# moss-lab/ScanFold

Hardware: AMD Instinct MI355X
Metric: windows/sec (W=120, step=1, 100 shuffles) (higher is better)
Workload: dtype int32 (int16 LDS storage) energies; f64 partition function

## Files before the change

scanfold_amd/csrc/sf_mfe_fast.hip.h:

```cpp
#pragma once
#include <type_traits>
#include "sf_energy.h"
#include "sf_pk16.h"

#define SF_FAST_NR 34
#ifndef SF_FAST_TINY_D0
#define SF_FAST_TINY_D0 10
#endif
#define SF_FAST_CHUNK_D0 36
#ifndef SF_FAST_UNPACK
#define SF_FAST_UNPACK 1
#endif
#ifndef SF_UNP_PB
#define SF_UNP_PB 4
#endif
#define SF_HELP_MERGE_MAXW 118
#define SF_DML_HELPER_BIAS_256 26
#define SF_DML_HELPER_BIAS_W200 50
#define SF_DML_HELPER_BIAS(ng, wt) ((ng) == 256 ? ((wt) == 200 ? SF_DML_HELPER_BIAS_W200 : SF_DML_HELPER_BIAS_256) : 100000)
#define SF_HELP_NB_128 4
#define SF_HELP_NB_128G 8
#define SF_HELP_NB_256 6
#define SF_INF16 30000
#define SF_FAST_THRESH 10000
// ... 799 lines not shown
  const int type = X.tPair[S[i] * 8 + S[j]];
  int ext;
  if (i > 1 && j < W) ext = tExt[SF_TIDX(type, S[i - 1], S[j + 1])];
  else if (i > 1) ext = X.tD5[type * 5 + S[i - 1]];
  else if (j < W) ext = X.tD3[type * 5 + S[j + 1]];
  else ext = 0;
  return v - ext - (type > 2 ? X.TAU : 0);
}

__device__ inline int sf_fast_traceback(const SfFastCtx &X, const int32_t *f5s, const int16_t *tExt, const int lane,
                                        int16_t *stI, int16_t *stJ, int16_t *stM, char *dbL) {
  const int W = X.W;
  const bool FOLD = X.fold != 0;
  const uint8_t *S = X.S;
  const SfDevParams *D = X.D;
#define TC(i, j) sf_fast_c(X, tExt, (i), (j))
#define TF(i, j) (((j) - (i) < SFD_TURN + 1) ? SF_INF16 : (int)X.fML[FBASE((j) - (i)) + (i)-1])
#define TPAIR(i, j) (((j) - (i)) <= X.maxd ? (int)X.tPair[S[i] * 8 + S[j]] : 0)
  for (int x = lane; x < W; x += 64) dbL[x] = '.';
  int sp = 0, bad = 0;
  stI[0] = 1; stJ[0] = (int16_t)W; stM[0] = 0; sp = 1;
  while (sp > 0 && !bad) {
    --sp;
    int i = stI[sp], j = stJ[sp];
    const int ml = stM[sp];
    bool have_pair = false;
    if (ml == 0) {
      while (j > 0 && f5s[j] == f5s[j - 1]) j--;
      if (j < SFD_TURN + 2) continue;
      const int fij = f5s[j];
      int found = -1;
      for (int base = j - SFD_TURN - 1; base >= 1 && found < 0; base -= 64) {
        const int k = base - lane;
        bool ok = false;
        if (k >= 1) {
          const int type = TPAIR(k, j);
          if (type) {
            int ext;
            if (k > 1 && j < W) ext = tExt[SF_TIDX(type, S[k - 1], S[j + 1])];
            else if (k > 1) ext = X.tD5[type * 5 + S[k - 1]];
            else if (j < W) ext = X.tD3[type * 5 + S[j + 1]];
            else ext = 0;
            ok = (fij == f5s[k - 1] + TC(k, j) + ext + (type > 2 ? X.TAU : 0));
          }
        }
        const unsigned long long m = __ballot(ok);
        if (m) found = base - (__ffsll(m) - 1);
      }
      if (found < 0) { bad = 1; break; }
      stI[sp] = 1; stJ[sp] = (int16_t)(found - 1); stM[sp] = 0; sp++;
      i = found;
      have_pair = true;
    } else {
      if (j - i < SFD_TURN + 1) { bad = 1; break; }
      while (j - i > SFD_TURN + 1 && TF(i, j - 1) < SF_INF16 && TF(i, j) == TF(i, j - 1) + X.MLbase) j--;
      while (j - i > SFD_TURN + 1 && TF(i + 1, j) < SF_INF16 && TF(i, j) == TF(i + 1, j) + X.MLbase) i++;
      const int fij = TF(i, j);
      const int type = TPAIR(i, j);
      int stem = 0;
      if (type) {
        if (i > 1 && j < W) stem = X.tM[SF_TIDX(type, S[i - 1], S[j + 1])];
        else if (i > 1) stem = X.tD5[type * 5 + S[i - 1]];
        else if (j < W) stem = X.tD3[type * 5 + S[j + 1]];
        stem += (type > 2 ? X.TAU : 0) + X.MLintern;
      }
      if (type && fij == TC(i, j) + stem) {
        have_pair = true;
      } else {
        int found = -1;
        for (int base = i + SFD_TURN + 1; base <= j - SFD_TURN - 2 && found < 0; base += 64) {
          const int k = base + lane;
          bool ok = false;
          if (k <= j - SFD_TURN - 2) {
            const int a = TF(i, k), b = TF(k + 1, j);
            ok = a < SF_INF16 && b < SF_INF16 && fij == a + b;
          }
          const unsigned long long m = __ballot(ok);
          if (m) found = base + (__ffsll(m) - 1);
        }
        if (found < 0) { bad = 1; break; }
        stI[sp] = (int16_t)i; stJ[sp] = (int16_t)found; stM[sp] = 1; sp++;
        stI[sp] = (int16_t)(found + 1); stJ[sp] = (int16_t)j; stM[sp] = 1; sp++;
      }
    }
    while (have_pair) {
      dbL[i - 1] = '(';
      dbL[j - 1] = ')';
      const int type = TPAIR(i, j);
      const int cij = TC(i, j);
      if (cij == sfd_hairpin(D, S, i, j, type)) break;
      const int d = j - i;
      const int umax = sfd_min(SFD_MAXLOOP, d - 2 - (SFD_TURN + 1));
      int found = -1;
      if (umax >= 0) {
        const int tmax = umax * 31 + umax;
        for (int base = 0; base <= tmax && found < 0; base += 64) {
          const int t = base + lane;
          const int u1 = t / 31, u2 = t - u1 * 31;
          bool ok = false;
          if (u1 + u2 <= umax) {
            const int p = i + 1 + u1, q = j - 1 - u2;
            const int t2 = TPAIR(p, q);
            if (t2)
              ok = (cij == sfd_intloop(D, u1, u2, type, sfd_rtype(t2), S[i + 1], S[j - 1], S[p - 1], S[q + 1]) + TC(p, q) +
                           ((X.sc && (u1 | u2) == 0) ? X.sc[i] + X.sc[i + 1] + X.sc[j - 1] + X.sc[j] : 0));
          }
          const unsigned long long m = __ballot(ok);
          if (m) found = base + (__ffsll(m) - 1);
        }
      }
      if (found >= 0) {
        const int u1 = found / 31, u2 = found - u1 * 31;
        i = i + 1 + u1;
        j = j - 1 - u2;
        continue;
      }
      const int tr = sfd_rtype(type);
      const int mm = X.MLclosing + X.tM[SF_TIDX(tr, S[j - 1], S[i + 1])] + (tr > 2 ? X.TAU : 0) + X.MLintern;
      int fk = -1;
      for (int base = i + 1 + SFD_TURN + 1; base <= j - 1 - SFD_TURN - 2 && fk < 0; base += 64) {
        const int k = base + lane;
        bool ok = false;
        if (k <= j - 1 - SFD_TURN - 2) {
          const int a = TF(i + 1, k), b = TF(k + 1, j - 1);
          ok = a < SF_INF16 && b < SF_INF16 && cij == a + b + mm;
        }
        const unsigned long long m = __ballot(ok);
        if (m) fk = base + (__ffsll(m) - 1);
      }
      if (fk < 0) { bad = 1; break; }
      stI[sp] = (int16_t)(i + 1); stJ[sp] = (int16_t)fk; stM[sp] = 1; sp++;
      stI[sp] = (int16_t)(fk + 1); stJ[sp] = (int16_t)(j - 1); stM[sp] = 1; sp++;
      break;
    }
  }
#undef TC
#undef TF
#undef TPAIR
  return bad;
}


template <int NQ>
__device__ __forceinline__ void sf_fast_exterior(const SfFastCtx &X, const int W, const int lane, const int seq,
                                                 int32_t *f5s, const int16_t *tExt, const int16_t *etab,
                                                 const int32_t *flag,
                                                 int16_t *stack_area, char *dbL, int32_t *__restrict__ out,
                                                 int *__restrict__ ovf_cnt, int *__restrict__ ovf_list,
                                                 const int trace_stride, char *__restrict__ db_out,
                                                 int *__restrict__ status) {
  const uint8_t *S = X.S;
  const uint8_t *tPair = X.tPair;
  int P[NQ], sj[NQ], sj1[NQ];
#pragma unroll
  for (int q = 0; q < NQ; q++) {
    const int j = lane + 64 * q + 1;
    P[q] = SF_FAST_BIG * 2;
    sj[q] = j <= W ? S[j] : 0;
    sj1[q] = j <= W ? S[j + 1] : 0;
  }
  int f5prev = 0;
  const bool want_trace = db_out && (seq % trace_stride) == 0;
  if (lane == 0) f5s[0] = 0;
  auto column_min = [&](const int jf) -> int {
    const int l = (jf - 1) & 63, q = (jf - 1) >> 6;
    int v = SF_LANE_READ(P[0], l);
#pragma unroll
    for (int qq = 1; qq < NQ; qq++) {
      const int vq = SF_LANE_READ(P[qq], l);
      if (q == qq) v = vq;
    }
    return v;
  };
  constexpr int PF = 8;
  int cb[PF][NQ];
  auto load_row = [&](const int i, int(&dst)[NQ]) {
#pragma unroll
    for (int q = 0; q < NQ; q++) {
      const int j = lane + 64 * q + 1;
      dst[q] = (i <= W - SFD_TURN - 1 && j <= W && i + SFD_TURN + 1 <= j) ? (int)(etab ? etab : X.cg)[SF_CGIDX(i, j)] : SF_INF16;
    }
  };
#pragma unroll
  for (int k = 0; k < PF; k++) load_row(1 + k, cb[k]);
#pragma unroll 1
  for (int i0 = 1; i0 <= W - SFD_TURN - 1; i0 += PF) {
#pragma unroll
    for (int k = 0; k < PF; k++) {
      const int i = i0 + k;
      if (i <= W - SFD_TURN - 1) {
        if (i >= 2) {
          f5prev = sfd_min(f5prev, column_min(i - 1));
          if (want_trace && lane == 0) f5s[i - 1] = f5prev;
        }
        if (etab || X.cg_ext) {
#pragma unroll
          for (int q = 0; q < NQ; q++) P[q] = sfd_min(P[q], f5prev + cb[k][q]);
        } else {
        const int si = S[i], sim1 = S[i - 1];
#pragma unroll
        for (int q = 0; q < NQ; q++) {
          const int j = lane + 64 * q + 1;
          if (j <= W && i + SFD_TURN + 1 <= j) {
            const int type = j - i <= X.maxd ? tPair[si * 8 + sj[q]] : 0;
            if (type) {
              int ext;
              if (i > 1 && j < W) ext = tExt[SF_TIDX(type, sim1, sj1[q])];
              else if (i > 1) ext = X.tD5[type * 5 + sim1];
              else if (j < W) ext = X.tD3[type * 5 + sj1[q]];
              else ext = 0;
              P[q] = sfd_min(P[q], f5prev + cb[k][q] + ext + (type > 2 ? X.TAU : 0));
            }
          }
        }
        }
        load_row(i + PF, cb[k]);
      }
    }
  }
  for (int jf = sfd_max(W - SFD_TURN - 1, 1); jf <= W; jf++) {
    f5prev = sfd_min(f5prev, column_min(jf));
    if (want_trace && lane == 0) f5s[jf] = f5prev;
  }
  SF_WAVE_SYNC();
  const int over = flag[0] || f5prev < SF_FAST_OVF;
  if (lane == 0) {
    out[seq] = f5prev;
    if (over) {
      const int k = atomicAdd(ovf_cnt, 1);
      ovf_list[k] = seq;
    }
  }
  if (db_out && !over && (seq % trace_stride) == 0) {
    int16_t *stI = stack_area;
    int16_t *stJ = stI + W + 8;
    int16_t *stM = stJ + W + 8;
    const int bad = sf_fast_traceback(X, f5s, tExt, lane, stI, stJ, stM, dbL);
    char *dst = db_out + (size_t)(seq / trace_stride) * (W + 1);
    for (int x = lane; x <= W; x += 64) dst[x] = x < W ? dbL[x] : 0;
    if (bad && lane == 0) atomicOr(status, 1);
  }
}

#define SF_DEFER_ROWS_256 3
template <int NQ>
struct SfTrail {
  int F[NQ];
  int f3n;
  int row;
};
template <int NQ>
__device__ __forceinline__ void sf_trail_load(const int16_t *cgp, const int W, const int lane, const int i, int (&c)[NQ]) {
#pragma unroll
  for (int q = 0; q < NQ; q++) {
    const int j = lane + 1 + 64 * q;
    c[q] = (i >= 1 && j <= W && i + SFD_TURN + 1 <= j) ? (int)cgp[SF_CGIDX(i, j)] : SF_INF16;
  }
}
template <int NQ>
__device__ __forceinline__ void sf_trail_row(SfTrail<NQ> &T, const int lane, const int i, const int (&c)[NQ]) {
  if (i < 1) return;
  int m = c[0] + T.F[0];
#pragma unroll
  for (int q = 1; q < NQ; q++) m = sfd_min(m, c[q] + T.F[q]);
  T.f3n = sfd_min(T.f3n, sf_wave_min(m));
  if (i >= 2) {
    const int l = (i - 2) & 63, h = (i - 2) >> 6;
#pragma unroll
    for (int q = 0; q < NQ; q++) T.F[q] = (lane == l && h == q) ? T.f3n : T.F[q];
  }
}
template <int NQ, int NR>
__device__ __forceinline__ void sf_trail_rows(SfTrail<NQ> &T, const int lane, const int nrows, const int (&c)[NR][NQ]) {
#pragma unroll
  for (int k = 0; k < NR; k++)
    if (k < nrows) sf_trail_row<NQ>(T, lane, T.row - k, c[k]);
  T.row -= nrows;
}
template <int NQ>
__device__ __forceinline__ void sf_trail_result(const SfTrail<NQ> &T, const int lane, const int seq, const int over,
                                                int32_t *__restrict__ out, int *__restrict__ ovf_cnt,
                                                int *__restrict__ ovf_list) {
  if (lane == 0) {
    out[seq] = T.f3n;
    if (over || T.f3n < SF_FAST_OVF) {
      const int k = atomicAdd(ovf_cnt, 1);
      ovf_list[k] = seq;
    }
  }
}


enum SfStep {
  SF_STEP_SIZED,
  SF_STEP_GUARDED,
  SF_STEP_UNSPLIT,
  SF_STEP_SPLIT,
  SF_STEP_SPLIT16,
  SF_STEP_SPLIT8,
  SF_STEP_NARROW,
};
template <SfStep K>
using SfStepTag = std::integral_constant<SfStep, K>;

__device__ __forceinline__ int16_t sf_poison16(const int poison, const int x) {
  const int k = poison == 5 ? 1 + (int)(((uint32_t)x * 2654435761u) >> 30) : poison;
  return (int16_t)(k == 1 ? -32768 : (k == 2 ? -28000 : (k == 3 ? 0 : 32767)));
}

template <int NG, int WT, bool MG = false, bool HC = false, bool PZ = false>
__global__ __launch_bounds__(2 * NG, SF_FAST_WAVES_PER_SIMD) void sf_mfe_fast_kernel(const uint8_t *__restrict__ seqs, int n, int Wrt,
                                                             const SfDevParams *__restrict__ D,
                                                             const SfFastParams *__restrict__ F,
                                                             const SfFastRows *__restrict__ Rows,
                                                             int16_t *__restrict__ cg_all, int32_t *__restrict__ out,
                                                             int *__restrict__ ovf_cnt, int *__restrict__ ovf_list,
                                                             int trace_stride, char *__restrict__ db_out,
                                                             int *__restrict__ status, int *__restrict__ work_ctr,
                                                             const char *__restrict__ cons_rows,
                                                             const int32_t *__restrict__ sc_rows, int poison) {
  constexpr int NT = 2 * NG;
  constexpr bool FOLD = (NG == 256);
  const int W = WT ? WT : Wrt;
  SF_DYN_SMEM(smem);
  const SfFastLayout Lo = sf_fast_layout(W, HC);
  SfFastCtx X;
  char *const hcC = (char *)(smem + Lo.off_hc);
  uint8_t *const hcP = (uint8_t *)hcC + (W + 2), *const hcE = hcP + (W + 2);
  int16_t *const scS = (int16_t *)(smem + Lo.off_hc + (((3 * (W + 2)) + 1) & ~1));
  X.hc.c = (HC && cons_rows) ? hcC : nullptr; X.hc.partner = hcP; X.hc.encl = hcE;
  X.sc = (HC && sc_rows) ? scS : nullptr;
  X.fML = (int16_t *)smem;
  X.CI = (int16_t *)(smem + Lo.off_ci);
  X.C1N = nullptr; X.CB = nullptr;
  X.BN = (int16_t *)(smem + Lo.off_c1n);
#ifdef SF_EMUL
  sf_emul_bn_base = (const char *)X.BN; sf_emul_ci_base = (const char *)X.CI;
#endif
  X.DMLr = nullptr;
  int16_t *tab = (int16_t *)(smem + Lo.off_tab);
  X.t23 = tab; X.tI = tab + 175 - 25; X.t1n = tab + 325 - 25; X.tM = tab + 475 - 25; X.tH = tab + 625 - 25;
  X.tE = tab + 775 - 25; X.cg_ext = 1;
  X.tStack = tab + 925; X.tD5 = tab + 989; X.tD3 = tab + 1029;
  uint8_t *tPair = (uint8_t *)(tab + 1069);
  X.tPair = tPair;
  uint8_t *tRPair = (uint8_t *)(tab + SF_FAST_TAB_OLD);
  int16_t *t23in = tab + SF_FAST_TAB_OLD + 32;
  X.tRPair = tRPair; X.t23in = t23in;
  int32_t *flag = (int32_t *)(smem + Lo.off_flag);
  uint8_t *S = (uint8_t *)(smem + Lo.off_S);
  X.S = S;
  X.D = D; X.F = F; X.R = Rows; X.W = W; X.fold = FOLD; X.maxd = D->max_pair_dist;
  constexpr bool MERGE = MG && (NG == 128);
  constexpr bool UNPK = SF_FAST_UNPACK && (NG == 128);
  constexpr bool LGLOOPS = MG && (NG == 128);
  constexpr int TBLK = WT > 0 ? 1 : (NG == 128 ? (MG ? 2 : 1) : 0);
  X.bn_dup = (NG == 128);
  uint8_t *const cell_list = (MG && W >= SF_HELP_MERGE_MAXW) ? (uint8_t *)((int16_t *)(smem + Lo.off_tab) + 1069 + 32 + 1)
                                                            : (uint8_t *)(smem + Lo.off_list);
  X.TAU = D->P.TerminalAU; X.MLbase = D->P.MLbase; X.MLclosing = D->P.MLclosing; X.MLintern = D->P.MLintern[1];
  int32_t *f5s = (int32_t *)(smem + Lo.off_ci);
  int16_t *tExt = (int16_t *)(smem + Lo.off_ci + (((W + 1) * 4 + 3) & ~3));

  const int tid = threadIdx.x;
  X.cg = cg_all + (size_t)sf_fast_scratch_slot(blockIdx.x, gridDim.x) * SF_CG_ENTRIES(W);
  for (int x = tid; x < 175; x += NT) {
    tab[x] = F->mm23[x];
    if (x < 150) {
      tab[175 + x] = F->mmI[25 + x]; tab[325 + x] = F->mm1n[25 + x]; tab[475 + x] = F->mmM[25 + x];
      tab[625 + x] = F->mmH[25 + x]; tab[775 + x] = F->mmExt[25 + x];
    }
  }
  for (int x = tid; x < 175; x += NT) t23in[x] = F->mm23in[x];
  for (int x = tid; x < 64; x += NT) { tab[925 + x] = F->stackT[x]; tPair[x] = F->pair[x]; tRPair[x] = F->rpair[x]; }
  for (int x = tid; x < 40; x += NT) { tab[989 + x] = F->d5[x]; tab[1029 + x] = F->d3[x]; }

  {
    int16_t *uni = tab + 1069 + 32 + 1;
    X.uNIN = uni;
    for (int x = tid; x < 128; x += NT) uni[x] = F->uni[x];
  }
  const int grp = SF_WAVE_UNIFORM(tid / NG);
  const int tg = tid - grp * NG;
  constexpr int CENTRE = (NG == 256) ? 128 : 32;
  constexpr bool SHARE = SF_DML_HELPER_BIAS(NG, WT) < 10000;
  constexpr bool DML2 = (NG == 128);
  const int OFFs = ((W + 1) >> 1) - CENTRE;
  const int OFF = (NG > 64) ? (OFFs + NG) & (NG - 1) : 0;
  const int v = (tg + OFF) & (NG - 1);
  constexpr int MAIN_LO = (NG == 256) ? 64 : 0, MAIN_HI = (NG == 256) ? 191 : 63;
  const bool can_split = (NG == 128 && W >= 64) || NG == 256;
  const int split_d0 = can_split ? ((sfd_max(sfd_max(SFD_MAXLOOP + 6, 2 * (MAIN_LO - 1 + OFFs)), 2 * (W - OFFs - MAIN_HI)) + 1) & ~1) : 1 << 30;
  constexpr bool NARROW = (NG == 256);
  const int narrow_d0 = (NARROW && can_split && W >= 168)
                            ? sfd_max(split_d0, (sfd_max(2 * (96 - 1 + OFFs), 2 * (W - OFFs - 159)) + 1) & ~1) : 1 << 30;

  constexpr int NQ = NG / 64;
  const bool sweeper = SF_WAVE_UNIFORM(tid >> 6) == (NG == 128 ? 3 : 7);
  const int n_split_steps = split_d0 < W ? (W - split_d0 + 1) / 2 : 0;
  constexpr int DROWS = (NG == 128 || WT != 200) ? 4 : SF_DEFER_ROWS_256;
  const int defer_need = n_split_steps > 0 ? (W - SFD_TURN - 1 + n_split_steps - 1) / n_split_steps : 0;
  const int defer_rows = sfd_min(defer_need, DROWS);
  const bool defer_on = n_split_steps >= 8 && defer_need <= 4;
  SfTrail<NQ> T;
#pragma unroll
  for (int q = 0; q < NQ; q++) T.F[q] = 0;
  T.f3n = 0; T.row = 0;

  int *const next_slot = (int *)(smem + Lo.off_next);
  int seq = blockIdx.x;
  while (seq < n) {
    const uint8_t *src = seqs + (size_t)seq * W;
    constexpr bool PINF = true;
    int tidf = tid;
    if (PINF) SF_PIN(tidf);
    __syncthreads();
    if (PZ) {
      for (int x = tid; x < Lo.off_tab / 2; x += NT) ((int16_t *)smem)[x] = sf_poison16(poison, x);
      if (HC) for (int x = tid; x < (Lo.total - Lo.off_hc) / 2; x += NT) ((int16_t *)(smem + Lo.off_hc))[x] = sf_poison16(poison, x);
      __syncthreads();
    }
    for (int x = tidf; x < W; x += NT) S[x + 1] = sf_encode_nt(src[x]);
    if (MG && W >= SF_HELP_MERGE_MAXW) for (int x = tidf; x < 128; x += NT) ((int16_t *)(smem + Lo.off_tab) + 1069 + 32 + 1)[x] = F->uni[x];
    for (int x = tidf; x < (Lo.off_tab - Lo.off_ci) / 4; x += NT) ((uint32_t *)X.CI)[x] = sf_pk(SF_INF16, SF_INF16);
    int fetched = 0;
    if (tid == 0) {
      S[0] = 0; S[W + 1] = 0; flag[0] = 0;
      fetched = (int)gridDim.x + atomicAdd(work_ctr, 1);
    }
    __syncthreads();
    if (HC) {
      if (cons_rows)
        for (int x = tid; x < W; x += NT) hcC[x + 1] = cons_rows[(size_t)seq * W + x];
      if (sc_rows)
        for (int x = tid; x < W; x += NT) scS[x + 1] = (int16_t)sfd_max(sfd_min(sc_rows[(size_t)seq * W + x], 30000), -30000);
      __syncthreads();
      if (cons_rows && tid == 0) flag[0] = sf_hc_parse8(W, hcC, hcP, hcE) ? 2 : 0;
      __syncthreads();
      if (cons_rows && flag[0] == 2) {
        if (tid == 0) { atomicOr(status, 2); out[seq] = 0; *next_slot = fetched; }
        __syncthreads();
        seq = *next_slot;
        continue;
      }
    }
    int next_seq = n;
    const bool trail_this = defer_on && !(db_out && (seq % trace_stride) == 0);
    if (sweeper) {
#pragma unroll
      for (int q = 0; q < NQ; q++) T.F[q] = 0;
      T.f3n = 0; T.row = trail_this ? W - SFD_TURN - 1 : 0;
    }
    int ovf = 0;
    uint32_t H[14];
    int dprev = SF_INF16;
    int fnb = SF_FAST_BIG;
#pragma unroll
    for (int k = 0; k < 14; k++) H[k] = (uint32_t)SF_INF16 | ((uint32_t)SF_INF16 << 16);

    int slot2 = (SFD_TURN + 1 + grp - 2) % SF_FAST_NR, slotd = (SFD_TURN + 1 + grp) % SF_FAST_NR;
    auto build_list = [&](const int dd0) {
      const int lane = tid & 63;
      const int d1 = dd0 + 1;
      const int iH = ((v - 64) & (NG - 1)) - (dd0 >> 1);
      const bool vA = (dd0 < W) && (iH >= 1) && (iH + dd0 <= W), vB = (d1 < W) && (iH >= 1) && (iH + d1 <= W);
      const int tA = (vA && dd0 <= X.maxd) ? X.tPair[S[iH] * 8 + S[iH + dd0]] : 0;
      const int tB = (vB && d1 <= X.maxd) ? X.tPair[S[iH] * 8 + S[iH + d1]] : 0;
      const unsigned long long mA = __ballot(tA != 0), mB = __ballot(tB != 0);
      const int cA = __popcll(mA);
      uint8_t *list = cell_list + (((dd0 >> 1) & 1) << 7);
      const unsigned long long below = (1ull << lane) - 1ull;
      if (tA) list[__popcll(mA & below)] = (uint8_t)iH;
      if (tB) list[cA + __popcll(mB & below)] = (uint8_t)(iH | 128);
      if (lane == 0) list[127] = (uint8_t)(cA + __popcll(mB));
    };
    SfHU HU;
    auto step = [&](const int d0, auto kind_tag) {
      constexpr SfStep KIND = decltype(kind_tag)::value;
      constexpr int LGC = KIND == SF_STEP_SPLIT16 ? 4 : (KIND == SF_STEP_SPLIT8 ? 3 : (KIND == SF_STEP_SPLIT && LGLOOPS ? 5 : 0));
      constexpr bool DO_G = KIND == SF_STEP_SIZED, DO_CH = KIND == SF_STEP_GUARDED;
      const int d = d0 + grp;
      if (d0 == SFD_TURN + 1 + 2 && tid == 0) *next_slot = fetched;
      if (d0 == SFD_TURN + 1 + 4) next_seq = SF_WAVE_UNIFORM(*next_slot);
      constexpr bool split = KIND >= SF_STEP_SPLIT;
      constexpr bool narrow = KIND == SF_STEP_NARROW;
      if (NARROW && d0 == narrow_d0) {
        uint32_t *const xa = (uint32_t *)X.BN;
        const int RWc = W - 4;
        if (tg >= 96 && tg < 160) {
#pragma unroll
          for (int k = 0; k < 14; k++) xa[(grp * 16 + k) * RWc + 100 + (tg - 96)] = H[k];
          xa[(grp * 16 + 14) * RWc + 100 + (tg - 96)] = (uint32_t)dprev;
          xa[(grp * 16 + 15) * RWc + 100 + (tg - 96)] = (uint32_t)fnb;
        }
        __syncthreads();
        if (tg >= 64 && tg < 128) {
#pragma unroll
          for (int k = 0; k < 14; k++) H[k] = xa[(grp * 16 + k) * RWc + 100 + (tg - 64)];
          dprev = (int)xa[(grp * 16 + 14) * RWc + 100 + (tg - 64)];
          fnb = (int)xa[(grp * 16 + 15) * RWc + 100 + (tg - 64)];
        }
        __syncthreads();
      }
      const bool helper = split && (NG == 256 ? (narrow ? tg < 64 : (tg < 64 || tg >= 192)) : tg >= 64);
      const int vh = NG == 256 ? (narrow ? v + 96 : (tg < 64 ? v + 64 : v - 64)) : v - 64;
      const int vm = narrow ? ((v + 32) & (NG - 1)) : v;
      constexpr bool DML4 = NARROW && (WT == 200);
      const bool dmlw = DML4 && narrow && tg >= 128;
      const int vd = tg >= 192 ? v - 96 : v - 32;
      const int i = (NARROW && !DML4 && narrow && tg >= 128) ? -1
                    : ((dmlw ? (vd & (NG - 1)) : (helper ? (vh & (NG - 1)) : vm)) - (d >> 1));
      const int dml_terms = d - 2 * SFD_TURN - 2;
      const int dml_cut = d - SFD_TURN - 1 - sfd_max(sfd_min(dml_terms / 2 - SF_DML_HELPER_BIAS(NG, WT), dml_terms), 0);
      const bool valid = (d < W) && (i >= 1) && (i + d <= W);
      int fpart = SF_FAST_BIG;
      int dec = SF_FAST_BIG, eh = SF_FAST_BIG, e0 = SF_FAST_BIG;
      SfPub pub;
      pub.a = pub.b = 0; pub.tau = 0; pub.type = 0;
      int dc[DROWS][NQ];
      const bool sweep_now = defer_on && sweeper && split && T.row > 0;
      const int sweep_rows = sweep_now ? sfd_max(sfd_min(defer_rows, T.row - (W - d0)), 0) : 0;
      if (sweep_now) {
#pragma unroll
        for (int k = 0; k < DROWS; k++)
          if (k < sweep_rows) sf_trail_load<NQ>(X.cg, W, tid & 63, T.row - k, dc[k]);
      }
      if (__ballot(valid)) {
        if (DO_G && d0 < 8) sf_fast_cell<true, WT, SF_SEC_ALL, false, FOLD, 1>(X, d, i, valid, slot2, slotd, H, HU, ovf, grp == 0, fnb, fpart, dec, eh, e0, dprev, pub);
        else if (DO_G && d0 < SF_FAST_TINY_D0) sf_fast_cell<true, WT, SF_SEC_ALL, false, FOLD, 5>(X, d, i, valid, slot2, slotd, H, HU, ovf, grp == 0, fnb, fpart, dec, eh, e0, dprev, pub);
        else if (DO_CH && d0 < SF_FAST_CHUNK_D0) sf_fast_cell<false, WT, SF_SEC_ALL, true, FOLD, SFD_MAXLOOP, TBLK>(X, d, i, valid, slot2, slotd, H, HU, ovf, grp == 0, fnb, fpart, dec, eh, e0, dprev, pub);
        else if (!split) sf_fast_cell<false, WT, SF_SEC_ALL, false, FOLD, SFD_MAXLOOP, TBLK, false, UNPK && KIND == SF_STEP_UNSPLIT>(X, d, i, valid, slot2, slotd, H, HU, ovf, grp == 0, fnb, fpart, dec, eh, e0, dprev, pub);
        else if (DML4 && narrow) {
          const int nmain = dml_terms / 5, cA = SFD_TURN + 1 + nmain, cB = cA + (dml_terms - nmain + 1) / 2;
          uint32_t *const xa = (uint32_t *)X.BN;
          if (dmlw) {
            const bool wB = tg >= 192;
            sf_fast_cell<false, WT, SF_SEC_DML, false, FOLD, SFD_MAXLOOP, TBLK>(X, d, i, valid, slot2, slotd, H, HU, ovf, false, fnb, fpart, dec, eh, e0, dprev, pub, wB ? cB : cA, wB ? (1 << 20) : cB - 1);
            if (valid) xa[(grp * 16 + (wB ? 1 : 0)) * (W - 4) + 100 + (tg & 63)] = (uint32_t)sfd_min(dec, 32000);
          } else if (!helper) {
            sf_fast_cell<false, WT, SF_SEC_P1 | SF_SEC_C0 | SF_SEC_DML | SF_SEC_PRE, false, FOLD, SFD_MAXLOOP, TBLK>(X, d, i, valid, slot2, slotd, H, HU, ovf, grp == 0, fnb, fpart, dec, eh, e0, dprev, pub, SFD_TURN + 1, cA - 1);
          } else {
            sf_fast_cell<false, WT, SF_SEC_HELP, false, FOLD, SFD_MAXLOOP, TBLK>(X, d, i, valid, slot2, slotd, H, HU, ovf, grp == 0, fnb, fpart, dec, eh, e0, dprev, pub);
            if (valid) X.BN[2 * (slotd * (W - 4) + i - 1)] = (int16_t)sfd_min(eh, 32000);
          }
        }
        else if (!helper) {
          if (SHARE) sf_fast_cell<false, WT, SF_SEC_P1 | SF_SEC_C0 | SF_SEC_DML | SF_SEC_PRE, false, FOLD, SFD_MAXLOOP, TBLK>(X, d, i, valid, slot2, slotd, H, HU, ovf, grp == 0, fnb, fpart, dec, eh, e0, dprev, pub, SFD_TURN + 1, dml_cut - 1);
          else {
            static_assert(SHARE || DML2, "a main wave either shares the multiloop split with its helpers (NG = 256) or runs it two cells per lane (NG = 128)");
            dec = sf_fast_dml2<WT, LGC>(X, d, tid & 63, i, valid);
            sf_fast_cell<false, WT, SF_SEC_P1 | SF_SEC_C0 | SF_SEC_PRE, false, FOLD, SFD_MAXLOOP, TBLK, false, UNPK && split>(X, d, i, valid, slot2, slotd, H, HU, ovf, grp == 0, fnb, fpart, dec, eh, e0, dprev, pub);
          }
        } else if (MERGE) {
          const int lane = tid & 63;
          const uint8_t *list = cell_list + (((d0 >> 1) & 1) << 7);
          const int cT = SF_WAVE_UNIFORM((int)list[127]);
          const int e = (grp << 6) + lane;
          if (SF_WAVE_UNIFORM(cT > (grp << 6))) {
            const bool vC = e < cT;
            const int ent = vC ? list[e] : 1;
            const int g = ent >> 7, iC = ent & 127;
            const int s2 = slot2 - grp < 0 ? slot2 - grp + SF_FAST_NR : slot2 - grp;
            const int sd0 = slotd - grp < 0 ? slotd - grp + SF_FAST_NR : slotd - grp;
            const int sd1 = sd0 + 1 >= SF_FAST_NR ? 0 : sd0 + 1;
            SfFastCtx Xh = X;
            Xh.BN = X.BN + 2 * g * (W - 4);
            sf_fast_cell<false, WT, SF_SEC_HELP, false, FOLD, SFD_MAXLOOP, TBLK, true>(Xh, d0 + g, iC, vC, s2, sd0, H, HU, ovf, false, fnb, fpart, dec, eh, e0, dprev, pub);
            if (vC) X.BN[2 * ((g ? sd1 : sd0) * (W - 4) + iC - 1)] = (int16_t)sfd_min(eh, 32000);
          }
        } else {
          if (SHARE) {
            sf_fast_cell<false, WT, SF_SEC_HELP | SF_SEC_DML, false, FOLD, SFD_MAXLOOP, TBLK>(X, d, i, valid, slot2, slotd, H, HU, ovf, grp == 0, fnb, fpart, dec, eh, e0, dprev, pub, dml_cut);
            if (valid) {
              X.BN[2 * (slotd * (W - 4) + i - 1)] = (int16_t)sfd_min(eh, 32000);
              X.CI[slotd * (W - 4) + i - 1] = (int16_t)sfd_min(dec, 32000);
            }
          } else {
            sf_fast_cell<false, WT, SF_SEC_HELP, false, FOLD, SFD_MAXLOOP, TBLK>(X, d, i, valid, slot2, slotd, H, HU, ovf, grp == 0, fnb, fpart, dec, eh, e0, dprev, pub);
            if (valid) X.BN[2 * (slotd * (W - 4) + i - 1)] = (int16_t)sfd_min(eh, 32000);
          }
        }
      }
      if (sweep_now && sweep_rows > 0) sf_trail_rows<NQ, DROWS>(T, tid & 63, sweep_rows, dc);
      if (MERGE && grp == 1 && tg >= 64 && d0 + 2 >= split_d0 && d0 + 2 < W) build_list(d0 + 2);
      if (split) {
        __syncthreads();
        if (!helper && !dmlw && __ballot(valid)) {
          if (valid) {
            eh = X.BN[2 * (slotd * (W - 4) + i - 1)];
            if (DML4 && narrow) {
              const uint32_t *const xa = (const uint32_t *)X.BN;
              dec = sfd_min(dec, sfd_min((int)xa[(grp * 16) * (W - 4) + 100 + (tg & 63)], (int)xa[(grp * 16 + 1) * (W - 4) + 100 + (tg & 63)]));
            } else if (SHARE) dec = sfd_min(dec, (int)X.CI[slotd * (W - 4) + i - 1]);
          }
          sf_fast_cell<false, WT, SF_SEC_FIN | SF_SEC_POST, false, FOLD, SFD_MAXLOOP, TBLK>(X, d, i, valid, slot2, slotd, H, HU, ovf, grp == 0, fnb, fpart, dec, eh, e0, dprev, pub);
        }
      }
      __syncthreads();
      if (grp == 0 && valid && !helper && !dmlw) {
        const int d1 = d0 + 1;
        const int16_t *pd = X.fML + FBASE(d1), *pe = X.fML + FBASE(d0);
        const bool ex0 = i + d1 <= W, ex1 = i >= 2;
        const int ia = i - 1, ib = ex1 ? i - 2 : 0;
        const int p0 = pd[ia], p1 = pd[ib], q0 = pe[i], q1 = pe[ia], q2 = pe[ib];
        const int v0 = sfd_min(p0, sfd_min(q0, q1) + X.MLbase), v1 = sfd_min(p1, sfd_min(q1, q2) + X.MLbase);
        if ((ex0 && v0 < SF_FAST_OVF) || (ex1 && v1 < SF_FAST_OVF)) ovf = 1;
        const int g0 = (ex0 && v0 <= SF_FAST_THRESH) ? v0 : SF_INF16, g1 = (ex1 && v1 <= SF_FAST_THRESH) ? v1 : SF_INF16;
        if (ex0) X.fML[FBASE(d1) + ia] = (int16_t)g0;
        fnb = sfd_min(g0, g1) + X.MLbase;
      }
      slot2 += 2; if (slot2 >= SF_FAST_NR) slot2 -= SF_FAST_NR;
      slotd += 2; if (slotd >= SF_FAST_NR) slotd -= SF_FAST_NR;
    };
    {
      int d0 = SFD_TURN + 1;
      for (; d0 < SF_FAST_TINY_D0 && d0 < W; d0 += 2) step(d0, SfStepTag<SF_STEP_SIZED>{});
      for (; d0 < SF_FAST_CHUNK_D0 && d0 < W; d0 += 2) step(d0, SfStepTag<SF_STEP_GUARDED>{});
      if constexpr (UNPK) {
#pragma unroll
        for (int x = 0; x < 27; x++) HU.v[x] = (short)((x & 1) ? (H[x >> 1] >> 16) : (H[x >> 1] & 0xffffu));
      }
      for (; d0 < split_d0 && d0 < W; d0 += 2) step(d0, SfStepTag<SF_STEP_UNSPLIT>{});
      if constexpr (LGLOOPS) {
        for (; d0 < W - 30 && d0 < W; d0 += 2) step(d0, SfStepTag<SF_STEP_SPLIT>{});
        for (; d0 < W - 14 && d0 < W; d0 += 2) step(d0, SfStepTag<SF_STEP_SPLIT16>{});
        for (; d0 < W; d0 += 2) step(d0, SfStepTag<SF_STEP_SPLIT8>{});
      }
      for (; d0 < (NARROW ? narrow_d0 : W) && d0 < W; d0 += 2) step(d0, SfStepTag<SF_STEP_SPLIT>{});
      if constexpr (NARROW)
        for (; d0 < W; d0 += 2) step(d0, SfStepTag<SF_STEP_NARROW>{});
    }

    if (ovf) flag[0] = 1;
    if (trail_this) {
      __syncthreads();
      if (sweeper) {
        while (T.row >= 1) {
          int tc[4][NQ];
#pragma unroll
          for (int k = 0; k < 4; k++) sf_trail_load<NQ>(X.cg, W, tid & 63, T.row - k, tc[k]);
          sf_trail_rows<NQ, 4>(T, tid & 63, sfd_min(4, T.row), tc);
        }
        sf_trail_result<NQ>(T, tid & 63, seq, flag[0], out, ovf_cnt, ovf_list);
      }
    } else {
    int tidn = tid;
    if (PINF && WT != 120) SF_PIN(tidn);
    for (int x = tidn; x < 200; x += NT) tExt[x] = F->mmExt[x];
    __syncthreads();
    int16_t *etab = nullptr;
    if (tid < 64)
      sf_fast_exterior<NG / 64>(X, W, tidn, seq, f5s, tExt, etab, flag, (int16_t *)(smem + Lo.off_cb),
                      (char *)(smem + Lo.off_cb + ((3 * (W + 8) * 2 + 3) & ~3)), out, ovf_cnt, ovf_list, trace_stride,
                      db_out, status);
    }
    seq = next_seq;
  }
#undef FBASE
#undef FLEN
}

#define SF_FAST_INSTANCES(X)                                                                          \
  X(128, 0, false, false, false) X(128, 0, true, false, false) X(128, 120, true, false, false)        \
  X(256, 200, false, false, false) X(256, 0, false, false, false)                                     \
  X(128, 0, false, true, false) X(128, 0, true, true, false) X(256, 0, false, true, false)            \
  X(128, 0, false, false, true) X(128, 0, true, false, true) X(128, 120, true, false, true)           \
  X(256, 200, false, false, true) X(256, 0, false, false, true)
struct SfFastInstance {
  int ng, wt;
  bool mg, hc, pz;
};
static inline SfFastInstance sf_fast_select(int W, bool hc, bool pz) {
  SfFastInstance s;
  s.ng = sf_fast_threads(W) / 2;
  s.wt = (!hc && (W == 120 || W == 200)) ? W : 0;
  s.mg = s.wt == 120 || W < SF_HELP_MERGE_MAXW;
  s.hc = hc;
  s.pz = pz;
  return s;
}
static inline hipError_t sf_fast_configure() {
  hipError_t e;
#define SF_X(NG, WT, MG, HC, PZ)                                                                                                  \
  e = hipFuncSetAttribute((const void *)sf_mfe_fast_kernel<NG, WT, MG, HC, PZ>, hipFuncAttributeMaxDynamicSharedMemorySize, 160 * 1024); \
  if (e != hipSuccess) return e;
  SF_FAST_INSTANCES(SF_X)
#undef SF_X
  return hipSuccess;
}

static inline void sf_fast_geometry(int W, int n_cu, int n, int *grid, int *threads, size_t *lds, size_t *scratch,
                                    bool hc = false) {
  const SfFastLayout L = sf_fast_layout(W, hc);
  const int nt = sf_fast_threads(W);
  int per_cu = (160 * 1024) / L.total;
  const int by_waves = (4 * SF_FAST_WAVES_PER_SIMD) / (nt / 64);
  if (per_cu > by_waves) per_cu = by_waves;
  if (per_cu < 1) per_cu = 1;
  long long gsz = (long long)n_cu * per_cu;
  if (gsz > n) gsz = n;
  *grid = (int)gsz;
  *threads = nt;
  *lds = (size_t)L.total;
  *scratch = (size_t)((gsz + 7) & ~7LL) * SF_CG_ENTRIES(W) * sizeof(int16_t);
}

template <typename... A>
static inline bool sf_fast_launch(bool hc, int poison, int grid, int threads, size_t lds, hipStream_t st, const uint8_t *seqs, int n,
                                  int W, A... args) {
  const SfFastInstance s = sf_fast_select(W, hc, poison != 0);
#define SF_X(NG, WT, MG, HC, PZ)                                                                                    \
  if (s.ng == NG && s.wt == WT && s.mg == MG && s.hc == HC && s.pz == PZ && threads == 2 * NG) {                    \
    SF_LAUNCH((sf_mfe_fast_kernel<NG, WT, MG, HC, PZ>), grid, 2 * NG, lds, st, seqs, n, W, args..., poison);         \
    return true;                                                                                                    \
  }
  SF_FAST_INSTANCES(SF_X)
#undef SF_X
  return false;
}
```

Before: 44510.

## Specialize split-phase step loops per wave role with compile-time role tags

For the 128-group kernel, the split-phase diagonal loops are now instantiated four times, once for each wave role (main/helper × even/odd group). Each wave branches on its uniform wave index into its own copy. Inside a copy, grp, helper and sweeper are compile-time constants, so dead branches and per-lane role checks can be removed and register pressure may drop. The cost is larger code size and instruction-cache pressure. It also adds extra trail-state zeroing for non-sweeper waves, and the MERGE list build no longer checks split_d0 when roles are active.

```diff
diff --git a/scanfold_amd/csrc/sf_mfe_fast.hip.h b/scanfold_amd/csrc/sf_mfe_fast.hip.h
--- a/scanfold_amd/csrc/sf_mfe_fast.hip.h
+++ b/scanfold_amd/csrc/sf_mfe_fast.hip.h
@@ -1125,6 +1125,15 @@
 };
 template <SfStep K>
 using SfStepTag = std::integral_constant<SfStep, K>;
+enum SfRole {
+  SF_ROLE_ALL,
+  SF_ROLE_MAIN_EVEN,
+  SF_ROLE_MAIN_ODD,
+  SF_ROLE_HELP_EVEN,
+  SF_ROLE_HELP_ODD,
+};
+template <SfRole R>
+using SfRoleTag = std::integral_constant<SfRole, R>;
 
 __device__ __forceinline__ int16_t sf_poison16(const int poison, const int x) {
   const int k = poison == 5 ? 1 + (int)(((uint32_t)x * 2654435761u) >> 30) : poison;
@@ -1177,6 +1186,7 @@
   constexpr bool MERGE = MG && (NG == 128);
   constexpr bool UNPK = SF_FAST_UNPACK && (NG == 128);
   constexpr bool LGLOOPS = MG && (NG == 128);
+  constexpr bool ROLE_LOOPS = (NG == 128);
   constexpr int TBLK = WT > 0 ? 1 : (NG == 128 ? (MG ? 2 : 1) : 0);
   X.bn_dup = (NG == 128);
   uint8_t *const cell_list = (MG && W >= SF_HELP_MERGE_MAXW) ? (uint8_t *)((int16_t *)(smem + Lo.off_tab) + 1069 + 32 + 1)
@@ -1298,13 +1308,21 @@
       if (lane == 0) list[127] = (uint8_t)(cA + __popcll(mB));
     };
     SfHU HU;
-    auto step = [&](const int d0, auto kind_tag) {
+    const int grp_wave = grp;
+    const bool sweeper_wave = sweeper;
+    auto step = [&](const int d0, auto kind_tag, auto role_tag) {
       constexpr SfStep KIND = decltype(kind_tag)::value;
+      constexpr SfRole ROLE = decltype(role_tag)::value;
+      constexpr bool ROLES = ROLE != SF_ROLE_ALL;
+      static_assert(!ROLES || (NG == 128 && KIND >= SF_STEP_SPLIT && KIND <= SF_STEP_SPLIT8), "roles: the narrow kernel's split steps");
+      const int grp = ROLES ? (int)(ROLE == SF_ROLE_MAIN_ODD || ROLE == SF_ROLE_HELP_ODD) : grp_wave;
+      const bool hwave = ROLES ? ROLE >= SF_ROLE_HELP_EVEN : tg >= 64;
+      const bool sweeper = ROLES ? ROLE == SF_ROLE_HELP_ODD : sweeper_wave;
       constexpr int LGC = KIND == SF_STEP_SPLIT16 ? 4 : (KIND == SF_STEP_SPLIT8 ? 3 : (KIND == SF_STEP_SPLIT && LGLOOPS ? 5 : 0));
       constexpr bool DO_G = KIND == SF_STEP_SIZED, DO_CH = KIND == SF_STEP_GUARDED;
       const int d = d0 + grp;
-      if (d0 == SFD_TURN + 1 + 2 && tid == 0) *next_slot = fetched;
-      if (d0 == SFD_TURN + 1 + 4) next_seq = SF_WAVE_UNIFORM(*next_slot);
+      if (!ROLES && d0 == SFD_TURN + 1 + 2 && tid == 0) *next_slot = fetched;
+      if (!ROLES && d0 == SFD_TURN + 1 + 4) next_seq = SF_WAVE_UNIFORM(*next_slot);
       constexpr bool split = KIND >= SF_STEP_SPLIT;
       constexpr bool narrow = KIND == SF_STEP_NARROW;
       if (NARROW && d0 == narrow_d0) {
@@ -1325,7 +1343,7 @@
         }
         __syncthreads();
       }
-      const bool helper = split && (NG == 256 ? (narrow ? tg < 64 : (tg < 64 || tg >= 192)) : tg >= 64);
+      const bool helper = split && (NG == 256 ? (narrow ? tg < 64 : (tg < 64 || tg >= 192)) : hwave);
       const int vh = NG == 256 ? (narrow ? v + 96 : (tg < 64 ? v + 64 : v - 64)) : v - 64;
       const int vm = narrow ? ((v + 32) & (NG - 1)) : v;
       constexpr bool DML4 = NARROW && (WT == 200);
@@ -1405,7 +1423,7 @@
         }
       }
       if (sweep_now && sweep_rows > 0) sf_trail_rows<NQ, DROWS>(T, tid & 63, sweep_rows, dc);
-      if (MERGE && grp == 1 && tg >= 64 && d0 + 2 >= split_d0 && d0 + 2 < W) build_list(d0 + 2);
+      if (MERGE && grp == 1 && hwave && (ROLES || d0 + 2 >= split_d0) && d0 + 2 < W) build_list(d0 + 2);
       if (split) {
         __syncthreads();
         if (!helper && !dmlw && __ballot(valid)) {
@@ -1437,21 +1455,38 @@
     };
     {
       int d0 = SFD_TURN + 1;
-      for (; d0 < SF_FAST_TINY_D0 && d0 < W; d0 += 2) step(d0, SfStepTag<SF_STEP_SIZED>{});
-      for (; d0 < SF_FAST_CHUNK_D0 && d0 < W; d0 += 2) step(d0, SfStepTag<SF_STEP_GUARDED>{});
+      constexpr SfRoleTag<SF_ROLE_ALL> all_roles{};
+      for (; d0 < SF_FAST_TINY_D0 && d0 < W; d0 += 2) step(d0, SfStepTag<SF_STEP_SIZED>{}, all_roles);
+      for (; d0 < SF_FAST_CHUNK_D0 && d0 < W; d0 += 2) step(d0, SfStepTag<SF_STEP_GUARDED>{}, all_roles);
       if constexpr (UNPK) {
 #pragma unroll
         for (int x = 0; x < 27; x++) HU.v[x] = (short)((x & 1) ? (H[x >> 1] >> 16) : (H[x >> 1] & 0xffffu));
       }
-      for (; d0 < split_d0 && d0 < W; d0 += 2) step(d0, SfStepTag<SF_STEP_UNSPLIT>{});
-      if constexpr (LGLOOPS) {
-        for (; d0 < W - 30 && d0 < W; d0 += 2) step(d0, SfStepTag<SF_STEP_SPLIT>{});
-        for (; d0 < W - 14 && d0 < W; d0 += 2) step(d0, SfStepTag<SF_STEP_SPLIT16>{});
-        for (; d0 < W; d0 += 2) step(d0, SfStepTag<SF_STEP_SPLIT8>{});
-      }
-      for (; d0 < (NARROW ? narrow_d0 : W) && d0 < W; d0 += 2) step(d0, SfStepTag<SF_STEP_SPLIT>{});
+      for (; d0 < split_d0 && d0 < W; d0 += 2) step(d0, SfStepTag<SF_STEP_UNSPLIT>{}, all_roles);
+      auto split_loops = [&](auto role_tag) {
+        if constexpr (LGLOOPS) {
+          for (; d0 < W - 30 && d0 < W; d0 += 2) step(d0, SfStepTag<SF_STEP_SPLIT>{}, role_tag);
+          for (; d0 < W - 14 && d0 < W; d0 += 2) step(d0, SfStepTag<SF_STEP_SPLIT16>{}, role_tag);
+          for (; d0 < W; d0 += 2) step(d0, SfStepTag<SF_STEP_SPLIT8>{}, role_tag);
+        }
+        for (; d0 < W; d0 += 2) step(d0, SfStepTag<SF_STEP_SPLIT>{}, role_tag);
+      };
+      if constexpr (ROLE_LOOPS) {
+        const int wave = SF_WAVE_UNIFORM(tid >> 6);
+        if (wave == 0) split_loops(SfRoleTag<SF_ROLE_MAIN_EVEN>{});
+        else if (wave == 2) split_loops(SfRoleTag<SF_ROLE_MAIN_ODD>{});
+        else if (wave == 1) split_loops(SfRoleTag<SF_ROLE_HELP_EVEN>{});
+        else split_loops(SfRoleTag<SF_ROLE_HELP_ODD>{});
+        if (wave != 3) {
+#pragma unroll
+          for (int q = 0; q < NQ; q++) T.F[q] = 0;
+          T.f3n = 0; T.row = 0;
+        }
+      } else {
+        for (; d0 < (NARROW ? narrow_d0 : W) && d0 < W; d0 += 2) step(d0, SfStepTag<SF_STEP_SPLIT>{}, all_roles);
+      }
       if constexpr (NARROW)
-        for (; d0 < W; d0 += 2) step(d0, SfStepTag<SF_STEP_NARROW>{});
+        for (; d0 < W; d0 += 2) step(d0, SfStepTag<SF_STEP_NARROW>{}, all_roles);
     }
 
     if (ovf) flag[0] = 1;
```

Measured after the change: 46030, median of 6. +3.4%, better.
